# ntu-caokun/DIRECT

Hardware: AMD Instinct MI355X
Metric: ddp_iterations_per_sec (higher is better)
Workload: dtype f64

## Files before the change

### direct_amd/csrc/ddp_wave.h

```cpp
#pragma once
#include <stdint.h>

#include "ddp_tables.h"
#include "sched_ticket.h"

#if defined(DIRECT_EMULATE)
#include <cmath>
#include <cstdio>
#include <cstdlib>
#include <cstring>
namespace direct {
using std::fabs; using std::fma; using std::fmax; using std::fmin; using std::log; using std::pow; using std::sqrt;
inline int& emu_lane() { static thread_local int l = 64; return l; }
template <typename T>
inline T* uniform_ptr(T* p) { return p; }
template <typename T>
inline T emu_uniform(T x, int line) {
  static thread_local unsigned char seen[4096][sizeof(double)];
  const int l = emu_lane();
  if (l >= 64) return x;
  unsigned char* ref = seen[line & 4095];
  if (l == 0) {
    std::memcpy(ref, &x, sizeof(T));
  } else if (std::memcmp(ref, &x, sizeof(T)) != 0 && !(x != x)) {
// ... 912 lines not shown
      k.n0 = n[0];
      k.n1 = n[1];
      k.n2 = n[2];
      k.o = n[3];
    }
    k.r = (pk & kRMask) - 1;
    k.a0 = (pk >> kRB) & kAMask;
    return k;
  }
  DDP_DEV Row3 row_ops(const Real* A, int pk) const {
    const Real* p = A + ((pk >> kRB) & kAMask);
    Row3 v;
    v.a = p[0];
    v.b = p[1];
    v.c = p[2];
    return v;
  }
  DDP_DEV Real row_dot(const RowK<Real>& k, const Row3& v) const { return fma(k.n2, v.c, fma(k.n1, v.b, k.n0 * v.a)); }
  DDP_DEV Real row_lin(const Real* A, const RowK<Real>& k) const {
    return k.n0 * A[k.a0] + k.n1 * A[k.a0 + 1] + k.n2 * A[k.a0 + 2];
  }
  DDP_DEV Real row_c(const Real* val, const RowK<Real>& k) const {
    return row_lin(val, k) + k.o - (Real)B.k.shift;
  }

  DDP_DEV Real ctrl_val(const Real* zz, const Real* tpw, int cr, int d) const {
    const int o = ctrl_off(cr);
    Real v = 0;
#pragma unroll
    for (int i = 0; i < 6; i++) {
      int e = i - o;
      v += L.WbE[cr * 6 + i] * tpw[e < 0 ? 0 : e] * zz[3 * i + d];
    }
    return v;
  }
  DDP_DEV Real ctrl_dval(const Real* zz, const Real* tpw, int cr, int d) const {
    const int o = ctrl_off(cr);
    Real v = 0;
#pragma unroll
    for (int i = 0; i < 6; i++) {
      int e = i - o - 1;
      v += L.WdE[cr * 6 + i] * tpw[e < 0 ? 0 : e] * zz[3 * i + d];
    }
    return v;
  }
  DDP_DEV Real next_x(const Real* zz, const Real* tpw, int a) const {
    const int c = a / 3, d = a % 3;
    Real acc = 0;
#pragma unroll
    for (int i = 0; i < 6; i++) acc += L.WbE[90 + c * 6 + i] * tpw[i < c ? 0 : i - c] * zz[3 * i + d];
    return acc;
  }
  DDP_DEV Real jerk_part(const Real* zz, const Real* tpw, int a9) const {
    const int a = a9 / 3, d = a9 % 3;
    Real acc = 0;
#pragma unroll
    for (int a2 = 0; a2 < 3; a2++) acc += L.Rc[a * 3 + a2] * tpw[a + a2 + 1] * zz[9 + 3 * a2 + d];
    return acc * zz[9 + a9];
  }
  DDP_DEV double knot_cost(Real T, const Real* qp) const {
    Real acc = 0;
#pragma unroll
    for (int a = 0; a < 9; a++) acc += qp[a];
    Real q = (Real)0.5 * (Real)B.k.w_snap * acc;
    if (B.k.time_power == 2) q += (Real)0.5 * T * (Real)B.k.w_time * T;
    else q += (Real)0.5 * (Real)B.k.w_time * T;
    return (double)q;
  }
  DDP_DEV double terminal_sq() {
    Real acc = 0;
#pragma unroll
    for (int a = 0; a < 9; a++) acc += L.z[a] * L.z[a];
    return (double)acc;
  }

  DDP_DEV void count_visits(int which, int n) const {
#if !defined(DIRECT_EMULATE)
    if (B.visits != nullptr && threadIdx.x == 0) atomicAdd(&B.visits[which], (unsigned long long)n);
#else
    (void)which; (void)n;
#endif
  }

  DDP_DEV void eval_sweep(int buf, bool do_roll) {
    PLV(LogProd<Real>, plog);
    PLV(Real, slog);
    PLV(Real, serr);
    PLV(int, nviol);
    PLV(int, npos);
    LANES { LV(plog).init(); LV(serr) = 0; LV(nviol) = 0; LV(npos) = 0; }
    const int infeas = DDP_UNIFORM_I(st.infeas);
    double qsum = 0.0;
    int neg = 0;
    PLV(Real, zr);
    PLA(St, plr, kNPL);
    int Pn = np_(0);
    LANES {
      LV(zr) = ldx(Xp(buf, 0), lane < 19 ? lane : 18);
      const int pend = 4 * Pn - 1;
      for (int i = 0; i < kNPL; i++) LV(plr)[i] = planes_(0)[lane + 64 * i < pend ? lane + 64 * i : pend];
    }
    for (int k = 0; k < N; k++) {
      const int P = Pn;
      PLA(Real, yv, RPL);
      LANES {
        const bool rolled = do_roll && k > 0 && lane < 9;
        if (lane < 19) L.z[lane] = rolled ? pair_round(L.ft[0].xnx[lane]) : LV(zr);
        for (int i = 0; i < kNPL; i++)
          if (lane + 64 * i < 4 * P) L.pl[lane + 64 * i] = (Real)LV(plr)[i];
        if (infeas) {
          const St* yk = Sp_(B.Y[buf], k);
          for (int i = 0; i < RPL; i++) {
            if (!slot_on(i, P)) continue;
            const int r = (row_pack(i, lane, P) & kRMask) - 1;
            LV(yv)[i] = (Real)yk[r >= 0 ? r : 0];
          }
        }
      }
      if (k + 1 < N) {
        Pn = np_(k + 1);
        LANES {
          LV(zr) = ldx(Xp(buf, k + 1), lane < 19 ? lane : 18);
          const int pend = 4 * Pn - 1;
          for (int i = 0; i < kNPL; i++) LV(plr)[i] = planes_(k + 1)[lane + 64 * i < pend ? lane + 64 * i : pend];
        }
      }
      WSYNC();
      const Real T = L.z[18];
      if (T < 0) neg = 1;
      LANES { if (lane < 8) L.tp[lane] = powi(T, lane); }
      WSYNC();
      LANES {
        if (lane < 45) L.val[lane] = ctrl_val(L.z, L.tp, lane / 3, lane % 3);
        else if (lane < 54) { if (do_roll) L.ft[0].xnx[lane - 45] = next_x(L.z, L.tp, lane - 45); }
        else if (lane < 63) L.ft[0].qp[lane - 54] = jerk_part(L.z, L.tp, lane - 54);
        else L.val[45] = T;
      }
      WSYNC();
      qsum += knot_cost(T, L.ft[0].qp);
      LANES {
        for (int i = 0; i < RPL; i++) {
          if (!slot_on(i, P)) continue;
          const RowK<Real> rk = row_slot(i, lane, P);
          const int r = rk.r;
          if (r >= 0) {
            Real c = row_c(L.val, rk);
            if (infeas) {
              Real y = LV(yv)[i];
              LV(plog).mul(y);
              LV(serr) += fabs(c + y);
            } else {
              LV(plog).mul(-c);
            }
            if (c >= (Real)2.0e-4) LV(nviol)++;
            if (c > (Real)0) LV(npos)++;
          }
        }
        LV(plog).norm();
        if (do_roll && lane < 9) stx(Xp(buf, k + 1), lane, L.ft[0].xnx[lane]);
      }
      WSYNC();
    }
    LANES {
      if (lane < 9) L.z[lane] = ldx(Xp(buf, N), lane) - (Real)B.xd[(size_t)b * 9 + lane];
    }
    WSYNC();
    const double pterm = terminal_sq();
    WSYNC();
    LANES { LV(slog) = LV(plog).value(); }
    st.costq = qsum;
    st.cost = qsum + 0.5 * B.k.w_term * pterm;
    st.sumlog = WAVE_SUM_D(slog);
    st.errsum = WAVE_SUM_D(serr);
    st.viol = WAVE_SUM_I(nviol);
    st.npos = WAVE_SUM_I(npos);
    st.neg_time = neg;
  }

  DDP_DEV void reset_filter() {
    double logcost = st.cost - st.mu * st.sumlog;
    double err = 0.0;
    if (st.infeas) {
      err = st.errsum;
      if (err < B.k.tol) err = 0.0;
    }
    st.logcost = logcost;
    st.err = err;
    double* f = B.filt + (size_t)b * B.fcap * 2;
    f[0] = logcost;
    f[1] = err;
    st.nfilter = 1;
    st.step = 0;
    st.fp_failed = 0;
  }

  DDP_DEV void line_init() {
    const St* T0 = B.T0 + (size_t)b * B.nmax;
    for (int l = 0; l < N; l++) {
      const int P = np_(l);
      Real pa[3], pn[3];
      for (int d = 0; d < 3; d++) {
        pa[d] = (l == 0) ? (Real)B.x0[(size_t)b * 9 + d] : (Real)B.seeds[((size_t)b * B.nmax + l) * 3 + d];
        pn[d] = (l == N - 1) ? (Real)B.xd[(size_t)b * 9 + d] : (Real)B.seeds[((size_t)b * B.nmax + l + 1) * 3 + d];
      }
      LANES { for (int e = lane; e < 4 * P; e += 64) L.pl[e] = planes_(l)[e]; }
      Real Tk = (Real)T0[l];
      int vio = 1, cnt = 0;
      while (vio && cnt <= 4) {
        const Real Tk2 = Tk * Tk, Tk3 = Tk2 * Tk, Tk4 = Tk3 * Tk, Tk5 = Tk4 * Tk;
        const Real g0 = (Real)10.0 / Tk3, g1 = (Real)-15.0 / Tk4, g2 = (Real)6.0 / Tk5;
        LANES {
          if (lane < 19) {
            const int a = lane / 3, d = lane % 3;
            Real v = 0;
            if (lane < 3) v = pa[d];
            else if (lane >= 9 && lane < 18) v = (a == 3 ? g0 : (a == 4 ? g1 : g2)) * (pn[d] - pa[d]);
            else if (lane == 18) v = Tk;
            L.z[lane] = v;
          }
          if (lane < 8) L.tp[lane] = powi(Tk, lane);
        }
        WSYNC();
        LANES {
          if (lane < 45) L.val[lane] = ctrl_val(L.z, L.tp, lane / 3, lane % 3);
          else if (lane == 63) L.val[45] = Tk;
        }
        WSYNC();
        PLV(int, bad);
        LANES {
          LV(bad) = 0;
          for (int i = 0; i < RPL; i++) {
            if (!slot_on(i, P)) continue;
            const RowK<Real> rk = row_slot(i, lane, P);
            if (rk.r >= 0 && !(row_c(L.val, rk) < (Real)0)) LV(bad) = 1;
          }
        }
        if (WAVE_ANY(bad)) {
          Tk = (Real)2 * Tk;
          cnt++;
        } else {
          vio = 0;
        }
        WSYNC();
      }
      LANES {
        if (lane >= 9 && lane < 18) stx(Xp(0, l), lane, L.z[lane]);
        if (lane == 18) stx(Xp(0, l), 18, Tk);
      }
      WSYNC();
    }
  }

  DDP_DEV void begin() {
    N = B.n_seg[b];
    int bad_sizes = (N < 1 || N > B.nmax) ? 1 : 0;
    if (!bad_sizes) {
      PLV(int, badp);
      LANES {
        LV(badp) = 0;
        for (int k = lane; k < N; k += 64) {
          const int np = np_(k);
          if (np < 1 || np > B.pmax || np > Lds::kPMax) LV(badp) = 1;
        }
      }
      bad_sizes = WAVE_ANY(badp);
    }
    if (bad_sizes) {
      N = 0;
      LANES {
        int* dst = (int*)&L.st;
        for (int e = lane; e < (int)(sizeof(TrajState) / 4); e += 64) dst[e] = 0;
      }
      WSYNC();
      st.rtn = -100;
      st.done = 1;
      st.line_failed = 1;
      return;
    }
    st.nseg = N;
    st.cur = 0;
    st.infeas = B.infeas_in ? (int)B.infeas_in[b] : 0;
    st.infeas_ref = st.infeas;
    st.line_failed = 1;
    const St* T0 = B.T0 + (size_t)b * B.nmax;
    LANES {
      if (lane < 9) stx(Xp(0, 0), lane, (Real)B.x0[(size_t)b * 9 + lane]);
      for (int k = lane; k < N; k += 64) {
        St* rec = Xp(0, k);
        Real T = T0[k];
        if (B.k.zero_init || (B.init_bez == nullptr && B.init_poly == nullptr)) {
          for (int a = 0; a < 9; a++) stx(rec, 9 + a, (Real)0);
        } else if (B.init_poly != nullptr) {
          const St* row = B.init_poly + ((size_t)b * B.nmax + k) * 18;
          for (int a = 0; a < 9; a++) stx(rec, 9 + a, (Real)row[9 + a]);
        } else {
          const St* row = B.init_bez + ((size_t)b * B.nmax + k) * 18;
          for (int i = 3; i < 6; i++)
            for (int d = 0; d < 3; d++) {
              Real acc = 0;
              for (int l = 0; l < 6; l++) acc += (Real)kBez2Mono[l][i] * (T * (Real)row[d * 6 + l]);
              stx(rec, 9 + (i - 3) * 3 + d, acc / powi(T, i));
            }
        }
        stx(rec, 18, T);
      }
    }
    if (!B.k.zero_init && B.k.line_init) line_init();
    for (int k = 0; k < N; k++) {
      const int nc = 6 * np_(k) + 55;
      LANES {
        for (int i = 0; i < RPL; i++) {
          int r = lane + 64 * i;
          if (r < nc) {
            Sp_(B.S[0], k)[r] = (St)0.1;
            Sp_(B.Y[0], k)[r] = (St)0.01;
          }
        }
      }
    }
    WSYNC();
    eval_sweep(0, true);
    if (B.k.line_init && st.npos == 0 && st.infeas) {
      st.infeas = 0;
      eval_sweep(0, false);
    }
    st.prev_cost = st.cost;
    st.nc0 = 6 * np_(0) + 55;
    st.mu = st.cost / (double)N / (double)st.nc0;
    reset_filter();
    st.reg = B.k.line_init ? 10 : 0;
    st.bp_failed = 0;
    st.opterr = 0.0;
    st.stepsize = 0.0;
    st.rtn = 0;
    st.iter = 0;
    st.done = 0;
    st.bp_no_upd = 0;
    st.no_upd = 0;
    st.fwd_passes = 0;
    LANES {
      if (lane == 0) {
        GainBase* g = &B.gbase[b];
        g->mu = 0.0;
        g->buf = -1;
        g->kreach = N;
      }
    }
  }

  struct BRec {
    Acc r[6];
  };
  struct BwdCtx {
    int regi, buf, infeas, klo;
    Acc lam, sig;
    Real mu, wsn;
    int Pn, Pnn;
    Acc emu_u;
    PLV(Real, e_mu);
    PLV(Acc, e_qu);
    PLV(Pre, pre);
    PLA(int, pkn, RPL);
    PLV(BRec, rc);
  };
#ifndef DDP_KSPLIT
#define DDP_KSPLIT (SHARE && RPL <= 4)
#endif
  static constexpr bool kSplit = DDP_KSPLIT;

  DDP_DEV BwdShare* bshare_slot() const { return (kSplit && B.bshare && B.self) ? &B.bshare[b] : nullptr; }
  DDP_DEV double* rec_ptr(int k) const { return B.brec + ((size_t)(unsigned)DDP_UNIFORM_I(b * B.nmax + k)) * kRecDoubles; }
  DDP_DEV int* flag_ptr(int k) const { return B.bflag + (size_t)(unsigned)DDP_UNIFORM_I(b * B.nmax + k); }
#if !defined(DIRECT_EMULATE)
  typedef unsigned int U4 __attribute__((ext_vector_type(4)));
  typedef double D2 __attribute__((ext_vector_type(2)));
  static __device__ __forceinline__ void drain_stores() { asm volatile("s_waitcnt vmcnt(0)" ::: "memory"); }
  DDP_DEV void rec_store(int k, const BRec& r, int lane) const {
    __amdgpu_buffer_rsrc_t rs = __builtin_amdgcn_make_buffer_rsrc(rec_ptr(k), 0, kRecDoubles * 8, 0x00020000);
#pragma unroll
    for (int p = 0; p < 3; p++) {
      D2 v;
      v.x = r.r[2 * p];
      v.y = r.r[2 * p + 1];
      __builtin_amdgcn_raw_buffer_store_b128(__builtin_bit_cast(U4, v), rs, (p * 64 + lane) * 16, 0, 16 );
    }
  }
  DDP_DEV void rec_load(int k, BRec& r, int lane) const {
    __amdgpu_buffer_rsrc_t rs = __builtin_amdgcn_make_buffer_rsrc(rec_ptr(k), 0, kRecDoubles * 8, 0x00020000);
#pragma unroll
    for (int p = 0; p < 3; p++) {
      const D2 v = __builtin_bit_cast(D2, __builtin_amdgcn_raw_buffer_load_b128(rs, (p * 64 + lane) * 16, 0, 16 ));
      r.r[2 * p] = v.x;
      r.r[2 * p + 1] = v.y;
    }
  }
  DDP_DEV void flag_set(int k, int tag) const {
    drain_stores();
    a_store(flag_ptr(k), tag);
  }
  DDP_DEV int flag_peek(int k) const { return __hip_atomic_load(flag_ptr(k), __ATOMIC_RELAXED, __HIP_MEMORY_SCOPE_AGENT); }
  DDP_DEV int flag_wait(int k, int tag) const {
    int spins = 0;
    while (a_load(flag_ptr(k)) != tag) {
      __builtin_amdgcn_s_sleep(1);
      if (++spins > kSpinLimit) {
        proto_error();
        return 0;
// ... 2395 lines not shown
```

### direct_amd/csrc/direct_ddp.hip

```cpp
#include <hip/hip_runtime.h>

#include <cmath>
#include <cstdio>
#include <cstdlib>
#include <cstring>
#include <string>
#include <vector>

#include "../../include/direct_ddp.h"
#include "ddp_wave.h"
#include "traj_sample.h"
#include "traj_eval.h"
#include "traj_audit.h"
#include "corridor_io.h"
#include "host_stage.h"
#include "rccl_gather.h"

using namespace direct;

#if defined(DDP_TIMING)
#undef DDP_TICK_OBJ
#define DDP_TICK_OBJ W
#endif
#ifndef DDP_WAVES_F32
#define DDP_WAVES_F32 1
#endif
#ifndef DDP_WAVES_F64
#define DDP_WAVES_F64 1
#endif
typedef double Cmp;
#ifndef DDP_WAVES_WIDE
#define DDP_WAVES_WIDE 2
#endif
#ifndef DDP_WAVES_WIDER
#define DDP_WAVES_WIDER 1
#endif
template <typename St>
struct MinWaves { static constexpr int v = DDP_WAVES_F32; };
template <>
struct MinWaves<double> { static constexpr int v = DDP_WAVES_F64; };

template <typename St>
__device__ __forceinline__ int traj_of(const Batch<St>& B, int i) {
  return B.idx ? __builtin_amdgcn_readfirstlane(B.idx[i]) : i;
}

template <typename St, int RPL>
__global__ __launch_bounds__(64) void k_begin(Batch<St> B) {
  __shared__ WaveLds<Cmp, St, RPL> lds;
  Wave<Cmp, St, RPL> W(B, lds, traj_of(B, blockIdx.x));
  W.init_tables();
  W.begin();
  W.store_state();
}

template <typename St, int RPL>
__global__ __launch_bounds__(64, (RPL > 7 ? DDP_WAVES_WIDER : (RPL > 4 ? DDP_WAVES_WIDE : MinWaves<St>::v))) void k_iterate(Batch<St> B, int n_iters) {
  __shared__ WaveLds<Cmp, St, RPL> lds;
  Wave<Cmp, St, RPL> W(B, lds, traj_of(B, blockIdx.x));
  W.load_state();
  if (__builtin_amdgcn_readfirstlane(lds.st.done)) return;
  W.init_tables();
  W.iterate(n_iters);
  W.store_state();
}

constexpr int kDoneBit = 1 << 30;
#ifndef DDP_POLL_SLEEP
#define DDP_POLL_SLEEP 32
#endif
struct Sched {
  unsigned* ticket;
  int* done_epoch;
  int* err;
  int chunk;
  int half;
  int prio;
  int tail;
  int* dbg;
#if defined(DDP_SCHED_DEBUG)
  int* mark;
  int grid;
#endif
  int* waves;
  int* alive;
  int yield_k, yield_min;
};
__device__ __attribute__((noinline)) int next_work(Sched S, HelpSlot* slots, BwdShare* sweeps, const int32_t* idx, sched::TicketPlan P, int held,
                                                   int* waited, int* help) {
  unsigned t = (unsigned)held;
  if (held < 0) {
    unsigned tv = 0;
    if (threadIdx.x == 0) tv = __hip_atomic_fetch_add(S.ticket, 1u, __ATOMIC_RELAXED, __HIP_MEMORY_SCOPE_AGENT);
    t = (unsigned)__builtin_amdgcn_readfirstlane((int)tv);
    *waited = 0;
  }
  *help = 0;
  if (t >= P.total_help) return -1;
  const sched::Ticket tk = sched::ticket_decode(P, t);
  const int e = tk.waits_for, bi = tk.slot;
  const int b = idx ? __builtin_amdgcn_readfirstlane(idx[bi]) : bi;
  int ready = (e == 0) ? 1 : 0, have = 0, wanted = 0;
  int spins = 0;
  const unsigned long long wait_t0 = __builtin_amdgcn_s_memrealtime();
#if defined(DDP_SCHED_DEBUG)
  if (S.mark != nullptr && threadIdx.x == 0) S.mark[blockIdx.x] = 60;
  if (!ready && threadIdx.x == 0) __hip_atomic_fetch_add(&S.dbg[12], 1, __ATOMIC_RELAXED, __HIP_MEMORY_SCOPE_AGENT);
  const int was_waiting = !ready;
#endif
  for (; !ready && !wanted && spins < kSpinLimit; spins++) {
#if defined(DDP_SCHED_DEBUG)
    if (spins == (1 << 18) && threadIdx.x == 0 && __hip_atomic_exchange(&S.dbg[23], 1, __ATOMIC_RELAXED, __HIP_MEMORY_SCOPE_AGENT) == 0) {
      S.dbg[16] = (int)t; S.dbg[17] = e; S.dbg[18] = S.done_epoch[b];
      S.dbg[19] = (int)__hip_atomic_load(S.ticket, __ATOMIC_RELAXED, __HIP_MEMORY_SCOPE_AGENT);
      S.dbg[20] = __hip_atomic_load(&S.dbg[12], __ATOMIC_RELAXED, __HIP_MEMORY_SCOPE_AGENT);
      S.dbg[21] = __hip_atomic_load(&S.dbg[13], __ATOMIC_RELAXED, __HIP_MEMORY_SCOPE_AGENT);
      S.dbg[22] = (int)((__builtin_amdgcn_s_memrealtime() - wait_t0) / 100000ull);
    }
#endif
    int hv = 0, g = 0, r = 0, lr = 0, sw = 0;
    if (threadIdx.x == 0) {
      hv = __hip_atomic_load(&S.done_epoch[b], __ATOMIC_RELAXED, __HIP_MEMORY_SCOPE_AGENT);
      if (slots) {
        g = __hip_atomic_load(&slots[b].gen, __ATOMIC_RELAXED, __HIP_MEMORY_SCOPE_AGENT);
        r = __hip_atomic_load(&slots[b].next_round, __ATOMIC_RELAXED, __HIP_MEMORY_SCOPE_AGENT);
        lr = __hip_atomic_load(&slots[b].last_round, __ATOMIC_RELAXED, __HIP_MEMORY_SCOPE_AGENT);
      }
      if (sweeps) {
        const unsigned w = __hip_atomic_load(&sweeps[b].word, __ATOMIC_RELAXED, __HIP_MEMORY_SCOPE_AGENT);
        const unsigned long long c = __hip_atomic_load(&sweeps[b].claim, __ATOMIC_RELAXED, __HIP_MEMORY_SCOPE_AGENT);
        sw = ((w >> kBsCountBits) != 0 && (int)(w & kBsCountMask) < kBsMaxHelpers &&
              (long long)(c & 0xffffffffull) < (long long)(c >> 32) - (long long)kClaimBias) ? 1 : 0;
      }
// ... 281 lines not shown
  } while (0)

struct direct_ddp_handle_s {
  int dtype = 0, device = 0, max_batch = 0, nmax = 0, pmax = 0, ncs = 0, rpl = 2, fcap = 0;
  struct Cls { int rpl, off, cnt; };
  std::vector<Cls> classes;
  int32_t* order = nullptr;
  int32_t* cls_dev = nullptr;
  int* tickets = nullptr;
  int slots_of[16] = {};
  int n_cu = 0;
  hipStream_t cstream[12] = {};
  hipEvent_t cev[12] = {}, fork_ev = nullptr;
  size_t rsz = 4;
  hipStream_t stream = nullptr;
  hipEvent_t ev0 = nullptr, ev1 = nullptr;
  hs::EventPair sample_ev, eval_ev, audit_ev;
  hs::Block eval_S;
  hs::Block audit_ws;
  hs::Block stage;
  int n_launches = 0;
  bool timed = false;
  void *x0 = nullptr, *xd = nullptr, *T0 = nullptr, *planes = nullptr, *init_bez = nullptr, *T_next = nullptr;
  void* init_poly = nullptr;
  void* seeds = nullptr;
  int32_t *n_seg = nullptr, *n_planes = nullptr;
  uint8_t *infeas_in = nullptr, *infeas_next = nullptr;
  void *X[direct::kMaxBuf] = {}, *S[direct::kMaxBuf] = {}, *Y[direct::kMaxBuf] = {};
  int nbuf = 3;
  HelpSlot* help = nullptr;
  bool small_dyn = true;
  int help_early = 1;
  int single_ratio = 8;
  int help_mode = -1;
  BwdShare* bshare = nullptr;
  int* bflag = nullptr;
  double* brec = nullptr;
  char *in_blob = nullptr, *out_blob = nullptr;
  char *in_host = nullptr, *out_host = nullptr, *out0_host = nullptr;
  size_t in_blob_bytes = 0, out_blob_bytes = 0;
  hipEvent_t in_ev = nullptr;
  bool in_ev_pending = false;
  char* batch_dev = nullptr;
  static constexpr int kBatchRing = 4;
  char* batch_pin = nullptr;
  hipEvent_t batch_ev[16][kBatchRing] = {};
  bool batch_ev_used[16][kBatchRing] = {};
  unsigned batch_seq[16] = {};
  int bshare_cap = 0;
  int bshare_mode = -1;
  void *KU = nullptr, *KS = nullptr, *KY = nullptr;
  double* filt = nullptr;
  TrajState* st = nullptr;
  GainBase* gbase = nullptr;
  void* fieldbuf = nullptr;
  size_t fieldbuf_bytes = 0;
  struct {
    int32_t *rtn, *iter_used, *fwd_passes;
    uint8_t *infeas_out, *line_failed_out;
    void *cost, *costq, *jerk_cost, *terminal_norm2, *opterr, *mu, *bez, *poly, *T;
  } o = {};
  int *best_idx = nullptr;
  double* best_cost = nullptr;
  void *g_recs = nullptr, *g_blocks = nullptr, *g_win = nullptr, *g_in = nullptr;
  int g_ranks = 0;
  int* sched = nullptr;
  int* live = nullptr;
  unsigned long long* visits = nullptr;
  direct_ddp_launch_info_t last_info = {};
  int sched_slots = 0;
  int slots_cap = 0;
  int sched_chunk = 1;
  int sched_half = -1;
  int pair_trials = -1;
  int sched_prio = 1;
  int sched_tail = 8;
  int yield_k = 0;
  int* nwaves = nullptr;
  int* sched_dbg = nullptr;
  int* sched_mark = nullptr;
  bool dynamic = true;
  int B = 0;
  bool begun = false;
  direct_ddp_params_t params = {};
  direct_ddp_batch_in_t cur_in = {};
  std::vector<void*> allocs;
};

template <typename T>
static direct_status_t dalloc(direct_ddp_handle_t h, T** p, size_t bytes) {
  hipError_t e = hs::alloc_all(h->allocs, {hs::want(p, bytes)});
  if (e != hipSuccess) return fail(DIRECT_ERR_DEVICE, std::string("hipMalloc: ") + hipGetErrorString(e));
  return DIRECT_OK;
}
#define TRY(expr)                            \
  do {                                       \
    direct_status_t s_ = (expr);             \
    if (s_ != DIRECT_OK) return s_;          \
  } while (0)

static std::vector<direct_ddp_handle_s::Cls> batch_classes(direct_ddp_handle_t h) {
  if (!h->classes.empty()) return h->classes;
  return {direct_ddp_handle_s::Cls{h->rpl, 0, h->B}};
}
template <typename Real>
static int resident_slots(direct_ddp_handle_t h, int rpl);

template <typename Real>
static Batch<Real> make_batch(direct_ddp_handle_t h, const direct_ddp_batch_in_t& in, const direct_ddp_params_t& p,
                              const direct_ddp_handle_s::Cls& c) {
  Batch<Real> B;
  memset(&B, 0, sizeof(B));
  B.B = c.cnt; B.idx = h->classes.empty() ? nullptr : h->order + c.off;
  B.nmax = h->nmax; B.pmax = h->pmax; B.ncs = h->ncs; B.fcap = h->fcap;
  B.n_seg = in.n_seg; B.x0 = (const Real*)in.x0; B.xd = (const Real*)in.xd; B.T0 = (const Real*)in.T0;
  B.n_planes = in.n_planes; B.planes = (const Real*)in.planes; B.init_bez = (const Real*)in.init_bez;
  B.init_poly = (const Real*)in.init_poly;
  B.seeds = (const Real*)in.seeds;
  B.infeas_in = in.infeas_in;
  for (int i = 0; i < h->nbuf; i++) {
    B.X[i] = (Real*)h->X[i]; B.S[i] = (Real*)h->S[i]; B.Y[i] = (Real*)h->Y[i];
  }
  B.nbuf = h->nbuf;
  B.help = nullptr;
  B.sched_err = h->sched + 1;
  B.visits = nullptr;
  B.live = nullptr;
  B.KU = (Real*)h->KU; B.KS = (Real*)h->KS; B.KY = (Real*)h->KY; B.filt = h->filt; B.st = h->st;
  B.gbase = h->gbase;
  SolveConst& k = B.k;
  k.max_vel = p.max_vel; k.max_acc = p.max_acc; k.w_snap = p.w_snap; k.w_term = p.w_terminal;
  k.w_time = p.w_time;
  k.reg_base = p.zero_init ? 1.6 : 4.0;
  k.shift = p.minvo ? 0.0 : 2.0e-4;
  k.tol = 1.0e-7;
  k.iter_max = p.iter_max; k.time_power = p.time_power; k.zero_init = p.zero_init;
  k.line_init = p.line_init; k.minvo = p.minvo; k.fixed_iters = p.fixed_iters; k.exact_dt = p.exact_dt;
  const int slots = resident_slots<Real>(h, c.rpl);
  k.pair_trials = h->pair_trials >= 0 ? h->pair_trials : 1;
  if (h->pair_trials < 0 && h->help && h->help_mode != 0 && h->dynamic && h->nmax >= 80 && (long long)c.cnt * h->single_ratio <= (long long)slots)
    k.pair_trials = 0;
  return B;
}

#if defined(DDP_DEV_RPL2)
#define RPL_LAUNCH(rpl, stream, KERNEL, Real, grid, ...) \
  hipLaunchKernelGGL((KERNEL<Real, 2>), dim3(grid), dim3(64), 0, stream, __VA_ARGS__)
#else
#define RPL_CASE(stream, KERNEL, Real, grid, R, ...) \
  case R: hipLaunchKernelGGL((KERNEL<Real, R>), dim3(grid), dim3(64), 0, stream, __VA_ARGS__); break;
#define RPL_LAUNCH(rpl, stream, KERNEL, Real, grid, ...)            \
  do {                                                              \
    switch (rpl) {                                                  \
      RPL_CASE(stream, KERNEL, Real, grid, 2, __VA_ARGS__)          \
      RPL_CASE(stream, KERNEL, Real, grid, 3, __VA_ARGS__)          \
      RPL_CASE(stream, KERNEL, Real, grid, 4, __VA_ARGS__)          \
      RPL_CASE(stream, KERNEL, Real, grid, 5, __VA_ARGS__)          \
      RPL_CASE(stream, KERNEL, Real, grid, 6, __VA_ARGS__)          \
      RPL_CASE(stream, KERNEL, Real, grid, 7, __VA_ARGS__)          \
      RPL_CASE(stream, KERNEL, Real, grid, 8, __VA_ARGS__)          \
      RPL_CASE(stream, KERNEL, Real, grid, 10, __VA_ARGS__)         \
      RPL_CASE(stream, KERNEL, Real, grid, 12, __VA_ARGS__)         \
      default: hipLaunchKernelGGL((KERNEL<Real, 14>), dim3(grid), dim3(64), 0, stream, __VA_ARGS__); \
    }                                                               \
  } while (0)
#endif

static int rpl_class(int slots) {
#if defined(DDP_DEV_RPL2)
  (void)slots;
  return 2;
#else
  return slots <= 2 ? 2 : (slots <= 8 ? slots : (slots <= 10 ? 10 : (slots <= 12 ? 12 : 14)));
#endif
}
template <typename Real>
static int resident_slots(direct_ddp_handle_t h, int rpl) {
  if (rpl < 0 || rpl > 15) return 0;
  if (h->slots_of[rpl] != 0) return h->slots_of[rpl] < 0 ? 0 : h->slots_of[rpl];
  int per_cu = 0;
  hipError_t e;
#if defined(DDP_DEV_RPL2)
  e = hipOccupancyMaxActiveBlocksPerMultiprocessor(&per_cu, k_iterate_dyn<Real, 2>, 64, 0);
#else
  switch (rpl) {
#define OCC_CASE(R) case R: e = hipOccupancyMaxActiveBlocksPerMultiprocessor(&per_cu, k_iterate_dyn<Real, R>, 64, 0); break;
    OCC_CASE(2) OCC_CASE(3) OCC_CASE(4) OCC_CASE(5) OCC_CASE(6) OCC_CASE(7) OCC_CASE(8) OCC_CASE(10) OCC_CASE(12)
#undef OCC_CASE
    default: e = hipOccupancyMaxActiveBlocksPerMultiprocessor(&per_cu, k_iterate_dyn<Real, 14>, 64, 0);
  }
#endif
  int v = (e == hipSuccess && per_cu > 0) ? per_cu * h->n_cu : 0;
  if (h->slots_cap > 0 && v > h->slots_cap) v = h->slots_cap;
  h->slots_of[rpl] = v > 0 ? v : -1;
  return v;
}

template <typename Real>
static void launch_begin_t(direct_ddp_handle_t h) {
  for (const auto& c : batch_classes(h)) {
    auto Bt = make_batch<Real>(h, h->cur_in, h->params, c);
    RPL_LAUNCH(c.rpl, h->stream, k_begin, Real, c.cnt, Bt);
  }
}
static hipStream_t class_stream(direct_ddp_handle_t h, size_t ci, size_t n_classes) {
  if (n_classes <= 1 || ci >= 12) return h->stream;
  if (!h->fork_ev && hipEventCreateWithFlags(&h->fork_ev, hipEventDisableTiming) != hipSuccess) return h->stream;
  if (!h->cstream[ci]) {
    if (hipStreamCreateWithFlags(&h->cstream[ci], hipStreamNonBlocking) != hipSuccess ||
        hipEventCreateWithFlags(&h->cev[ci], hipEventDisableTiming) != hipSuccess) {
      h->cstream[ci] = nullptr;
      return h->stream;
    }
  }
  return h->cstream[ci];
}
template <typename Real>
static void launch_iterate_t(direct_ddp_handle_t h, int n, int mode) {
  const auto classes = batch_classes(h);
  (void)hipMemsetAsync(h->visits, 0, 4 * sizeof(unsigned long long), h->stream);
  direct_ddp_launch_info_t& li = h->last_info;
  li = direct_ddp_launch_info_t{};
  li.n_buffers = h->nbuf; li.batch = h->B;
  if (mode == 0) {
    (void)hipMemsetAsync(h->tickets, 0, 16 * sizeof(int), h->stream);
    (void)hipMemsetAsync(h->sched + 2, 0, (size_t)h->B * sizeof(int), h->stream);
    if (h->help) (void)hipMemsetAsync(h->help, 0, (size_t)h->B * sizeof(HelpSlot), h->stream);
    if (h->bshare && h->bshare_mode != 0) {
      const size_t nb = (size_t)(h->B < h->bshare_cap ? h->B : h->bshare_cap);
      (void)hipMemsetAsync(h->bshare, 0, nb * sizeof(BwdShare), h->stream);
      (void)hipMemsetAsync(h->bflag, 0, nb * h->nmax * sizeof(int), h->stream);
    }
  }
  bool forked = false;
  if (mode == 0 && classes.size() > 1 && class_stream(h, 0, classes.size()) != h->stream) {
    (void)hipEventRecord(h->fork_ev, h->stream);
    forked = true;
  }
  int biggest = -1;
  for (size_t ci = 0; ci < classes.size(); ci++) {
    const auto& c = classes[ci];
    auto Bt = make_batch<Real>(h, h->cur_in, h->params, c);
    Bt.visits = h->visits;
#if defined(DDP_TIMELINE)
    if (g_tl_n < (size_t)h->B * kTimelineDepth * 4) {
      if (g_tl) (void)hipFree(g_tl);
      g_tl_n = (size_t)h->B * kTimelineDepth * 4;
      (void)hipMalloc((void**)&g_tl, g_tl_n * 8);
    }
    (void)hipMemsetAsync(g_tl, 0, (size_t)h->B * kTimelineDepth * 4 * 8, h->stream);
    Bt.tl = g_tl;
#endif
    hipStream_t st = h->stream;
    if (forked) {
      st = class_stream(h, ci, classes.size());
      if (st != h->stream) (void)hipStreamWaitEvent(st, h->fork_ev, 0);
    }
    if (mode != 0) {
      RPL_LAUNCH(c.rpl, st, k_pass, Real, c.cnt, Bt, mode);
      continue;
    }
    const int slots = resident_slots<Real>(h, c.rpl);
    const bool help = h->help && (h->help_mode >= 0 ? h->help_mode != 0 : (2 * c.cnt <= 3 * slots && (h->nmax >= 80 || 8 * c.cnt <= slots)));
    const bool is_big = biggest < 0 || c.cnt > classes[biggest].cnt;
    if (is_big) {
      biggest = (int)ci;
      li.pair_trials = Bt.k.pair_trials; li.resident_waves = slots; li.dynamic = 0; li.shared_search = 0; li.single_steps = 0; li.half_tickets = 0;
      li.shared_sweep = 0;
    }
    const bool sweep_ok = h->bshare != nullptr && c.rpl <= 4 && h->B <= h->bshare_cap;
    static_assert(sizeof(Batch<Real>) <= 1024, "Batch grew past its device-copy slot");
    auto publish = [&](Batch<Real>& Bb) {
      if (ci >= 16 || h->batch_pin == nullptr) { Bb.bshare = nullptr; return; }
      const int slot = (int)(h->batch_seq[ci]++ % direct_ddp_handle_s::kBatchRing);
      if (h->batch_ev_used[ci][slot]) (void)hipEventSynchronize(h->batch_ev[ci][slot]);
      char* stage = h->batch_pin + ((size_t)ci * direct_ddp_handle_s::kBatchRing + slot) * 1024;
      Bb.self = h->batch_dev + ci * 1024;
      memcpy(stage, &Bb, sizeof(Bb));
      (void)hipMemcpyAsync(h->batch_dev + ci * 1024, stage, sizeof(Bb), hipMemcpyHostToDevice, st);
      if (h->batch_ev[ci][slot] == nullptr && hipEventCreateWithFlags(&h->batch_ev[ci][slot], hipEventDisableTiming) != hipSuccess) {
        h->batch_ev[ci][slot] = nullptr;
        (void)hipStreamSynchronize(st);
        h->batch_ev_used[ci][slot] = false;
      } else {
        (void)hipEventRecord(h->batch_ev[ci][slot], st);
        h->batch_ev_used[ci][slot] = true;
      }
    };
    if (sweep_ok && h->bshare_mode == 2) {
      Bt.bshare = h->bshare; Bt.bflag = h->bflag; Bt.brec = h->brec; Bt.bforce = 1; Bt.bvisits = h->visits + 2;
      if (is_big) li.shared_sweep = 2;
    }
    if (h->dynamic && slots > 0 && (c.cnt > slots || (help && h->small_dyn))) {
      Sched S;
      S.ticket = (unsigned*)(h->tickets + (ci < 16 ? ci : 15));
      S.err = h->sched + 1;
      S.done_epoch = h->sched + 2;
      S.half = h->sched_half > 0 ? 1 : 0;
      S.chunk = S.half ? 1 : h->sched_chunk;
      S.prio = h->sched_prio;
      S.tail = help ? h->sched_tail : 0;
      S.dbg = h->sched_dbg;
#if defined(DDP_SCHED_DEBUG)
      S.mark = nullptr; S.grid = slots;
      if (slots <= 8192) { S.mark = h->sched_mark; Bt.mark = h->sched_mark; (void)hipMemsetAsync(h->sched_mark, 0, 2 * 8192 * sizeof(int), st); }
#endif
      S.waves = h->nwaves + (ci < 16 ? ci : 15);
      S.alive = h->live + (ci < 16 ? ci : 15);
      S.yield_k = h->yield_k;
      S.yield_min = 64;
      if (h->yield_k > 0) {
        S.tail = 0;
        (void)hipMemsetD32Async((hipDeviceptr_t)S.waves, slots, 1, st);
        (void)hipMemsetD32Async((hipDeviceptr_t)S.alive, c.cnt, 1, st);
      }
      if (help) {
        Bt.help = h->help;
        Bt.help_early = h->help_early;
        int* live = h->live + (ci < 16 ? ci : 15);
        (void)hipMemsetD32Async((hipDeviceptr_t)live, c.cnt, 1, st);
        Bt.live = live;
        Bt.tail_thresh = h->single_ratio > 0 ? slots / h->single_ratio : 0;
        if (is_big) { li.shared_search = 1; li.single_steps = Bt.k.pair_trials ? 0 : 1; }
        if (sweep_ok && h->bshare_mode != 0 && h->bshare_mode != 2 && S.chunk == 1 && (h->bshare_mode > 0 || 8 * c.cnt <= slots)) {
          Bt.bshare = h->bshare; Bt.bflag = h->bflag; Bt.brec = h->brec; Bt.bforce = 0; Bt.bvisits = h->visits + 2;
          if (is_big) li.shared_sweep = 1;
        }
      }
      if (is_big) { li.dynamic = 1; li.half_tickets = S.half; }
      if (Bt.bshare) {
        publish(Bt);
        switch (c.rpl) {
          case 2: hipLaunchKernelGGL((k_iterate_dyn<Real, 2, true>), dim3(slots), dim3(64), 0, st, Bt, n, S); break;
#if !defined(DDP_DEV_RPL2)
          case 3: hipLaunchKernelGGL((k_iterate_dyn<Real, 3, true>), dim3(slots), dim3(64), 0, st, Bt, n, S); break;
          default: hipLaunchKernelGGL((k_iterate_dyn<Real, 4, true>), dim3(slots), dim3(64), 0, st, Bt, n, S);
#endif
        }
      } else {
        RPL_LAUNCH(c.rpl, st, k_iterate_dyn, Real, slots, Bt, n, S);
      }
    } else {
      Bt.bshare = nullptr;
      if (is_big && li.shared_sweep) li.shared_sweep = 0;
      RPL_LAUNCH(c.rpl, st, k_iterate, Real, c.cnt, Bt, n);
    }
    {
      auto Bs = make_batch<Real>(h, h->cur_in, h->params, c);
      Bs.visits = h->visits;
      RPL_LAUNCH(c.rpl, st, k_stuck, Real, c.cnt, Bs);
    }
    if (forked && st != h->stream) {
      (void)hipEventRecord(h->cev[ci], st);
      (void)hipStreamWaitEvent(h->stream, h->cev[ci], 0);
    }
  }
}
template <typename Real>
static void launch_field_t(direct_ddp_handle_t h, int field, int set) {
  for (const auto& c : batch_classes(h)) {
    auto Bt = make_batch<Real>(h, h->cur_in, h->params, c);
    RPL_LAUNCH(c.rpl, h->stream, k_field, Real, c.cnt, Bt, field, (Real*)h->fieldbuf, set);
  }
}
template <typename Real>
static OutPtrs<Real> out_ptrs(direct_ddp_handle_t h, const direct_ddp_batch_out_t* out) {
  OutPtrs<Real> O;
  const bool dev = out->mem == DIRECT_MEM_DEVICE;
#define PICK(f) (dev ? out->f : (out->f ? h->o.f : nullptr))
  O.rtn = PICK(rtn); O.iter_used = PICK(iter_used); O.fwd_passes = PICK(fwd_passes);
  O.infeas_out = PICK(infeas_out); O.line_failed_out = PICK(line_failed_out);
  O.cost = (Real*)PICK(cost); O.costq = (Real*)PICK(costq); O.jerk_cost = (Real*)PICK(jerk_cost);
  O.terminal_norm2 = (Real*)PICK(terminal_norm2); O.opterr = (Real*)PICK(opterr); O.mu = (Real*)PICK(mu);
  O.bez = (Real*)PICK(bez); O.poly = (Real*)PICK(poly); O.T = (Real*)PICK(T);
#undef PICK
  return O;
}
template <typename Real>
static void launch_finish_t(direct_ddp_handle_t h, const direct_ddp_batch_out_t* out) {
  auto O = out_ptrs<Real>(h, out);
  for (const auto& c : batch_classes(h)) {
    auto Bt = make_batch<Real>(h, h->cur_in, h->params, c);
    RPL_LAUNCH(c.rpl, h->stream, k_finish, Real, c.cnt, Bt, O, (const int*)(h->sched + 1));
  }
}

static direct_status_t staged_upload(direct_ddp_handle_t h, hs::Stage& st, const char* name) {
  const hipError_t e = hs::stage_upload(st, h->stage, h->stream);
  return e == hipSuccess ? DIRECT_OK : fail(DIRECT_ERR_DEVICE, std::string(name) + ": staging: " + hipGetErrorString(e));
}
static direct_status_t staged_finish(direct_ddp_handle_t h, const hs::Stage& st, const char* name) {
  hipError_t e = hs::stage_download(st, h->stream, hipGetLastError());
  if (st.host) e = hs::drain(h->stream, e);
  return e == hipSuccess ? DIRECT_OK : fail(DIRECT_ERR_DEVICE, std::string(name) + ": " + hipGetErrorString(e));
}
static direct_status_t workspace(direct_ddp_handle_t h, hs::Block& ws, size_t bytes, const char* name) {
  const hipError_t e = hs::grow(ws, h->stream, bytes);
  return e == hipSuccess ? DIRECT_OK : fail(DIRECT_ERR_DEVICE, std::string("workspace of ") + name + ": " + hipGetErrorString(e));
}

template <typename Real>
static direct_status_t sample_t(direct_ddp_handle_t h, const direct_sample_in_t* in, direct_sample_out_t* out) {
  const size_t B = in->batch, nm = in->n_seg_max, cap = in->capacity, r = sizeof(Real);
  SampleArgs<Real> A;
// ... 1022 lines not shown
```

Baseline: 2.590 million.

## Fold scheduler resets into begin kernel and fuse S/Y init into first sweep

Replaces the many per-launch hipMemsetAsync calls that clear tickets, help slots, bshare flags and counters with a single reset kernel. When a begin launch has just run, those resets are done inside k_begin itself, so no separate clear is needed before the next iterate. It also fuses the S/Y initialisation loop into the first eval_sweep, caches row_pack results across knots, reuses ctrl_val for next_x, and trims k_begin's LDS to raise occupancy. The costs are more complex clean-state bookkeeping on the host and a risk of stale state if the flags fall out of sync with the actual buffers.

```diff
diff --git a/direct_amd/csrc/ddp_wave.h b/direct_amd/csrc/ddp_wave.h
--- a/direct_amd/csrc/ddp_wave.h
+++ b/direct_amd/csrc/ddp_wave.h
@@ -1018,7 +1018,7 @@
 #endif
   }
 
-  DDP_DEV void eval_sweep(int buf, bool do_roll) {
+  DDP_DEV void eval_sweep(int buf, bool do_roll, bool init_sy) {
     PLV(LogProd<Real>, plog);
     PLV(Real, slog);
     PLV(Real, serr);
@@ -1028,37 +1028,49 @@
     const int infeas = DDP_UNIFORM_I(st.infeas);
     double qsum = 0.0;
     int neg = 0;
+    set_sweep_ptrs(buf);
+    const Real y_init = (Real)(St)0.01;
     PLV(Real, zr);
     PLA(St, plr, kNPL);
-    int Pn = np_(0);
+    PLA(int, pkv, RPL);
+    int Ppk = -1;
+    int Pn = DDP_UNIFORM_I(npU(0));
     LANES {
-      LV(zr) = ldx(Xp(buf, 0), lane < 19 ? lane : 18);
+      LV(zr) = ldx(XpU(0, 0), lane < 19 ? lane : 18);
+      GCSt* pk = planesU(0);
       const int pend = 4 * Pn - 1;
-      for (int i = 0; i < kNPL; i++) LV(plr)[i] = planes_(0)[lane + 64 * i < pend ? lane + 64 * i : pend];
+      for (int i = 0; i < kNPL; i++) LV(plr)[i] = pk[lane + 64 * i < pend ? lane + 64 * i : pend];
     }
     for (int k = 0; k < N; k++) {
       const int P = Pn;
       PLA(Real, yv, RPL);
+      if (P != Ppk) {
+        LANES { for (int i = 0; i < RPL; i++) LV(pkv)[i] = row_pack(i, lane, P); }
+        Ppk = P;
+      }
       LANES {
         const bool rolled = do_roll && k > 0 && lane < 9;
         if (lane < 19) L.z[lane] = rolled ? pair_round(L.ft[0].xnx[lane]) : LV(zr);
         for (int i = 0; i < kNPL; i++)
           if (lane + 64 * i < 4 * P) L.pl[lane + 64 * i] = (Real)LV(plr)[i];
-        if (infeas) {
-          const St* yk = Sp_(B.Y[buf], k);
+        if (init_sy) {
+          for (int i = 0; i < RPL; i++) LV(yv)[i] = y_init;
+        } else if (infeas) {
+          GCSt* yk = SpU(sp.Y[0], k);
           for (int i = 0; i < RPL; i++) {
             if (!slot_on(i, P)) continue;
-            const int r = (row_pack(i, lane, P) & kRMask) - 1;
+            const int r = (LV(pkv)[i] & kRMask) - 1;
             LV(yv)[i] = (Real)yk[r >= 0 ? r : 0];
           }
         }
       }
       if (k + 1 < N) {
-        Pn = np_(k + 1);
+        Pn = DDP_UNIFORM_I(npU(k + 1));
         LANES {
-          LV(zr) = ldx(Xp(buf, k + 1), lane < 19 ? lane : 18);
+          LV(zr) = ldx(XpU(0, k + 1), lane < 19 ? lane : 18);
+          GCSt* pk = planesU(k + 1);
           const int pend = 4 * Pn - 1;
-          for (int i = 0; i < kNPL; i++) LV(plr)[i] = planes_(k + 1)[lane + 64 * i < pend ? lane + 64 * i : pend];
+          for (int i = 0; i < kNPL; i++) LV(plr)[i] = pk[lane + 64 * i < pend ? lane + 64 * i : pend];
         }
       }
       WSYNC();
@@ -1067,9 +1079,11 @@
       LANES { if (lane < 8) L.tp[lane] = powi(T, lane); }
       WSYNC();
       LANES {
-        if (lane < 45) L.val[lane] = ctrl_val(L.z, L.tp, lane / 3, lane % 3);
-        else if (lane < 54) { if (do_roll) L.ft[0].xnx[lane - 45] = next_x(L.z, L.tp, lane - 45); }
-        else if (lane < 63) L.ft[0].qp[lane - 54] = jerk_part(L.z, L.tp, lane - 54);
+        if (lane < 54) {
+          const Real v = ctrl_val(L.z, L.tp, lane / 3, lane % 3);
+          if (lane < 45) L.val[lane] = v;
+          else if (do_roll) L.ft[0].xnx[lane - 45] = v;
+        } else if (lane < 63) L.ft[0].qp[lane - 54] = jerk_part(L.z, L.tp, lane - 54);
         else L.val[45] = T;
       }
       WSYNC();
@@ -1077,7 +1091,7 @@
       LANES {
         for (int i = 0; i < RPL; i++) {
           if (!slot_on(i, P)) continue;
-          const RowK<Real> rk = row_slot(i, lane, P);
+          const RowK<Real> rk = row_unpack2(LV(pkv)[i]);
           const int r = rk.r;
           if (r >= 0) {
             Real c = row_c(L.val, rk);
@@ -1093,12 +1107,24 @@
           }
         }
         LV(plog).norm();
-        if (do_roll && lane < 9) stx(Xp(buf, k + 1), lane, L.ft[0].xnx[lane]);
+        if (do_roll && lane < 9) stx(XpU(0, k + 1), lane, L.ft[0].xnx[lane]);
+        if (init_sy) {
+          GSt* sk = SpU(sp.S[0], k);
+          GSt* yk = SpU(sp.Y[0], k);
+          const int nc = 6 * P + 55;
+          for (int i = 0; i < RPL; i++) {
+            const int r = lane + 64 * i;
+            if (r < nc) {
+              sk[r] = (St)0.1;
+              yk[r] = (St)0.01;
+            }
+          }
+        }
       }
       WSYNC();
     }
     LANES {
-      if (lane < 9) L.z[lane] = ldx(Xp(buf, N), lane) - (Real)B.xd[(size_t)b * 9 + lane];
+      if (lane < 9) L.z[lane] = ldx(XpU(0, N), lane) - (Real)B.xd[(size_t)b * 9 + lane];
     }
     WSYNC();
     const double pterm = terminal_sq();
@@ -1242,23 +1268,11 @@
       }
     }
     if (!B.k.zero_init && B.k.line_init) line_init();
-    for (int k = 0; k < N; k++) {
-      const int nc = 6 * np_(k) + 55;
-      LANES {
-        for (int i = 0; i < RPL; i++) {
-          int r = lane + 64 * i;
-          if (r < nc) {
-            Sp_(B.S[0], k)[r] = (St)0.1;
-            Sp_(B.Y[0], k)[r] = (St)0.01;
-          }
-        }
-      }
-    }
     WSYNC();
-    eval_sweep(0, true);
+    eval_sweep(0, true, true);
     if (B.k.line_init && st.npos == 0 && st.infeas) {
       st.infeas = 0;
-      eval_sweep(0, false);
+      eval_sweep(0, false, false);
     }
     st.prev_cost = st.cost;
     st.nc0 = 6 * np_(0) + 55;
diff --git a/direct_amd/csrc/direct_ddp.hip b/direct_amd/csrc/direct_ddp.hip
--- a/direct_amd/csrc/direct_ddp.hip
+++ b/direct_amd/csrc/direct_ddp.hip
@@ -46,9 +46,61 @@
 }
 
 template <typename St, int RPL>
-__global__ __launch_bounds__(64) void k_begin(Batch<St> B) {
-  __shared__ WaveLds<Cmp, St, RPL> lds;
+struct BeginLds {
+  typedef WaveLds<Cmp, St, RPL> Lds;
+  static constexpr size_t kBytes = (offsetof(Lds, ft) + offsetof(typename Lds::FwdT, G) + 15) / 16 * 16;
+  static_assert(offsetof(Lds, ft) > offsetof(Lds, G) && offsetof(Lds, ft) > offsetof(Lds, lt16), "k_begin's LDS head must hold the tables");
+  static_assert(RPL > 4 || kBytes <= 10 * 1024, "k_begin: sixteen workgroups per CU need at most 10 KB of LDS each");
+};
+struct SchedReset {
+  int* tickets;
+  int* done_epoch;
+  int* live;
+  int* nwaves;
+  unsigned long long* visits;
+  HelpSlot* help;
+  BwdShare* bshare;
+  int* bflag;
+  int nb_share, nmax;
+  int per_traj;
+  int cls0, n_cls;
+  int cnt[16], slots[16];
+};
+__device__ __forceinline__ void sched_reset(const SchedReset& R, int b, bool launch_part) {
+  const int lane = threadIdx.x;
+  if (R.per_traj) {
+    if (lane == 0) R.done_epoch[b] = 0;
+    if (R.help != nullptr) {
+      int* p = (int*)&R.help[b];
+      for (int e = lane; e < (int)(sizeof(HelpSlot) / 4); e += 64) p[e] = 0;
+    }
+    if (R.bshare != nullptr && b < R.nb_share) {
+      int* p = (int*)&R.bshare[b];
+      if (lane < (int)(sizeof(BwdShare) / 4)) p[lane] = 0;
+      int* f = R.bflag + (size_t)b * R.nmax;
+      for (int e = lane; e < R.nmax; e += 64) f[e] = 0;
+    }
+  }
+  if (launch_part) {
+    if (lane < R.n_cls) {
+      const int ci = R.cls0 + lane;
+      R.tickets[ci] = 0;
+      R.live[ci] = R.cnt[ci];
+      R.nwaves[ci] = R.slots[ci];
+    }
+    if (R.visits != nullptr && lane < 4) R.visits[lane] = 0ull;
+  }
+}
+static_assert(sizeof(BwdShare) / 4 <= 64 && sizeof(HelpSlot) % 4 == 0 && sizeof(BwdShare) % 4 == 0, "sched_reset clears these word by word");
+__global__ __launch_bounds__(64) void k_sched_reset(SchedReset R) { sched_reset(R, (int)blockIdx.x, blockIdx.x == 0); }
+
+template <typename St, int RPL>
+__global__ __launch_bounds__(64, (RPL > 4 ? 1 : 4)) void k_begin(Batch<St> B, SchedReset R) {
+  typedef BeginLds<St, RPL> Head;
+  __shared__ alignas(16) unsigned char head[Head::kBytes];
+  typename Head::Lds& lds = *reinterpret_cast<typename Head::Lds*>(head);
   Wave<Cmp, St, RPL> W(B, lds, traj_of(B, blockIdx.x));
+  sched_reset(R, W.b, blockIdx.x == 0);
   W.init_tables();
   W.begin();
   W.store_state();
@@ -496,6 +548,8 @@
   bool dynamic = true;
   int B = 0;
   bool begun = false;
+  bool sched_clean = false;
+  bool visits_clean = false;
   direct_ddp_params_t params = {};
   direct_ddp_batch_in_t cur_in = {};
   std::vector<void*> allocs;
@@ -611,11 +665,39 @@
 }
 
 template <typename Real>
+static SchedReset make_reset(direct_ddp_handle_t h, const std::vector<direct_ddp_handle_s::Cls>& classes, bool per_traj, bool visits) {
+  SchedReset R;
+  memset(&R, 0, sizeof(R));
+  R.tickets = h->tickets; R.done_epoch = h->sched + 2; R.live = h->live; R.nwaves = h->nwaves;
+  R.visits = visits ? h->visits : nullptr;
+  R.help = h->help;
+  if (h->bshare && h->bshare_mode != 0) {
+    R.bshare = h->bshare; R.bflag = h->bflag;
+    R.nb_share = h->B < h->bshare_cap ? h->B : h->bshare_cap;
+  }
+  R.nmax = h->nmax;
+  R.per_traj = per_traj ? 1 : 0;
+  R.cls0 = 0;
+  R.n_cls = (int)(classes.size() < 16 ? classes.size() : 16);
+  for (int ci = 0; ci < R.n_cls; ci++) {
+    R.cnt[ci] = classes[ci].cnt;
+    R.slots[ci] = resident_slots<Real>(h, classes[ci].rpl);
+  }
+  return R;
+}
+template <typename Real>
 static void launch_begin_t(direct_ddp_handle_t h) {
-  for (const auto& c : batch_classes(h)) {
+  const auto classes = batch_classes(h);
+  SchedReset R = make_reset<Real>(h, classes, true, true);
+  for (size_t ci = 0; ci < classes.size(); ci++) {
+    const auto& c = classes[ci];
     auto Bt = make_batch<Real>(h, h->cur_in, h->params, c);
-    RPL_LAUNCH(c.rpl, h->stream, k_begin, Real, c.cnt, Bt);
-  }
+    R.cls0 = (int)(ci < 16 ? ci : 15); R.n_cls = 1;
+    RPL_LAUNCH(c.rpl, h->stream, k_begin, Real, c.cnt, Bt, R);
+    R.visits = nullptr;
+  }
+  h->sched_clean = true;
+  h->visits_clean = true;
 }
 static hipStream_t class_stream(direct_ddp_handle_t h, size_t ci, size_t n_classes) {
   if (n_classes <= 1 || ci >= 12) return h->stream;
@@ -632,19 +714,17 @@
 template <typename Real>
 static void launch_iterate_t(direct_ddp_handle_t h, int n, int mode) {
   const auto classes = batch_classes(h);
-  (void)hipMemsetAsync(h->visits, 0, 4 * sizeof(unsigned long long), h->stream);
   direct_ddp_launch_info_t& li = h->last_info;
   li = direct_ddp_launch_info_t{};
   li.n_buffers = h->nbuf; li.batch = h->B;
-  if (mode == 0) {
-    (void)hipMemsetAsync(h->tickets, 0, 16 * sizeof(int), h->stream);
-    (void)hipMemsetAsync(h->sched + 2, 0, (size_t)h->B * sizeof(int), h->stream);
-    if (h->help) (void)hipMemsetAsync(h->help, 0, (size_t)h->B * sizeof(HelpSlot), h->stream);
-    if (h->bshare && h->bshare_mode != 0) {
-      const size_t nb = (size_t)(h->B < h->bshare_cap ? h->B : h->bshare_cap);
-      (void)hipMemsetAsync(h->bshare, 0, nb * sizeof(BwdShare), h->stream);
-      (void)hipMemsetAsync(h->bflag, 0, nb * h->nmax * sizeof(int), h->stream);
-    }
+  {
+    const bool need_sched = mode == 0 && !h->sched_clean;
+    if (need_sched || !h->visits_clean) {
+      const SchedReset R = make_reset<Real>(h, classes, need_sched, !h->visits_clean);
+      hipLaunchKernelGGL(k_sched_reset, dim3(need_sched ? h->B : 1), dim3(64), 0, h->stream, R);
+    }
+    if (mode == 0) h->sched_clean = false;
+    h->visits_clean = false;
   }
   bool forked = false;
   if (mode == 0 && classes.size() > 1 && class_stream(h, 0, classes.size()) != h->stream) {
@@ -725,15 +805,11 @@
       S.yield_min = 64;
       if (h->yield_k > 0) {
         S.tail = 0;
-        (void)hipMemsetD32Async((hipDeviceptr_t)S.waves, slots, 1, st);
-        (void)hipMemsetD32Async((hipDeviceptr_t)S.alive, c.cnt, 1, st);
       }
       if (help) {
         Bt.help = h->help;
         Bt.help_early = h->help_early;
-        int* live = h->live + (ci < 16 ? ci : 15);
-        (void)hipMemsetD32Async((hipDeviceptr_t)live, c.cnt, 1, st);
-        Bt.live = live;
+        Bt.live = h->live + (ci < 16 ? ci : 15);
         Bt.tail_thresh = h->single_ratio > 0 ? slots / h->single_ratio : 0;
         if (is_big) { li.shared_search = 1; li.single_steps = Bt.k.pair_trials ? 0 : 1; }
         if (sweep_ok && h->bshare_mode != 0 && h->bshare_mode != 2 && S.chunk == 1 && (h->bshare_mode > 0 || 8 * c.cnt <= slots)) {
```

Result: no change. 2.609 million (median of 6 runs) (+0.8%).
